# supabase/etl

Hardware: AMD Instinct MI355X
Metric: WAL bytes/s decoded (higher is better)
Workload: dtype u8; 1 GPU; cfg2_fixed_5xint4: 64 MiB batches of CopyData-framed pgoutput, device-resident in / device-resident out, offsets sidecar, NO_CONTROL | ASYNC; batch_bytes=67108819, frames_per_batch=594511, pool_batches=6, parallelism=shard1

## Files before the change

### etl_amd/csrc/plan.hip

```cpp
#include "lookback.hip.h"

namespace etlg {

struct WinLds {
  const ETLG_LDS_AS u8* base;
  DEV uint32_t w(uint32_t aoff) const { return ETLG_LDS_LD32(base + aoff); }
};
struct WinGlb {
  const u8* base; uint32_t lim;
  DEV uint32_t w(uint32_t aoff) const {
    uint32_t v = 0;
    if (aoff + 4 <= lim) __builtin_memcpy(&v, base + aoff, 4);
    else for (uint32_t k = 0; aoff + k < lim; k++) v |= (uint32_t)base[aoff + k] << (8 * k);
    return v;
  }
};
template <class M> DEV uint32_t rd32(const M& m, uint32_t off) {
  const uint32_t a = off & ~3u, s = off & 3u;
  return __builtin_amdgcn_alignbyte(m.w(a + 4), m.w(a), s);
}
template <class M> DEV uint64_t rd64(const M& m, uint32_t off) {
  const uint32_t a = off & ~3u, s = off & 3u;
  const uint32_t w0 = m.w(a), w1 = m.w(a + 4), w2 = m.w(a + 8);
  return __builtin_amdgcn_alignbyte(w1, w0, s) | ((uint64_t)__builtin_amdgcn_alignbyte(w2, w1, s) << 32);
// ... 10 lines not shown
  const int32_t sh = (int32_t)k - (int32_t)(4 * j);
  const uint32_t part = 0xFFFFFFFFu << (8 * ((uint32_t)sh & 3u));
  const uint32_t keep = sh <= 0 ? 0xFFFFFFFFu : sh >= 4 ? 0u : part;
  return (w & keep) | (0x30303030u & ~keep);
}

template <class M>
DEV uint64_t plan_int(const M& m, uint32_t cs, uint32_t n, uint32_t c0, uint32_t cls, uint32_t& ok) {
  const uint32_t neg = c0 == '-' ? 1u : 0u;
  const uint32_t sg = (c0 == '-' || c0 == '+') ? 1u : 0u;
  const uint32_t nd = n - sg;
  uint32_t bad = 0;
  uint64_t mag;
  if (cls == ETLG_TC_I64) {
    const uint32_t nn = n < 20u ? n : 20u;
    const uint32_t s0 = cs + nn - 20u, a = s0 & ~3u, s = s0 & 3u, k = 20u - (nd < 20u ? nd : 20u);
    const uint32_t w0 = m.w(a), w1 = m.w(a + 4), w2 = m.w(a + 8), w3 = m.w(a + 12), w4 = m.w(a + 16), w5 = m.w(a + 20);
    const uint32_t d0 = dig4(pad_word(__builtin_amdgcn_alignbyte(w1, w0, s), k, 0), bad);
    const uint32_t d1 = dig4(pad_word(__builtin_amdgcn_alignbyte(w2, w1, s), k, 1), bad);
    const uint32_t d2 = dig4(pad_word(__builtin_amdgcn_alignbyte(w3, w2, s), k, 2), bad);
    const uint32_t d3 = dig4(pad_word(__builtin_amdgcn_alignbyte(w4, w3, s), k, 3), bad);
    const uint32_t d4 = dig4(pad_word(__builtin_amdgcn_alignbyte(w5, w4, s), k, 4), bad);
    mag = (uint64_t)(d0 * 10000u + d1) * 1000000000000ull + (uint64_t)(d2 * 10000u + d3) * 10000ull + d4;
    const uint64_t lim = neg ? (1ull << 63) : (1ull << 63) - 1;
    ok = (n != 0u) & (nd != 0u) & (n <= 20u) & (nd <= 19u) & (bad == 0u) & (mag <= lim);
  } else {
    const uint32_t nn = n < 12u ? n : 12u;
    const uint32_t s0 = cs + nn - 12u, a = s0 & ~3u, s = s0 & 3u, k = 12u - (nd < 12u ? nd : 12u);
    const uint32_t w0 = m.w(a), w1 = m.w(a + 4), w2 = m.w(a + 8), w3 = m.w(a + 12);
    const uint32_t d0 = dig4(pad_word(__builtin_amdgcn_alignbyte(w1, w0, s), k, 0), bad);
    const uint32_t d1 = dig4(pad_word(__builtin_amdgcn_alignbyte(w2, w1, s), k, 1), bad);
    const uint32_t d2 = dig4(pad_word(__builtin_amdgcn_alignbyte(w3, w2, s), k, 2), bad);
    mag = (uint64_t)d0 * 100000000ull + (d1 * 10000u + d2);
    uint64_t lim;
    if (cls == ETLG_TC_U32) lim = 0xFFFFFFFFull;
    else if (cls == ETLG_TC_I16) lim = neg ? 0x8000ull : 0x7FFFull;
    else lim = neg ? 0x80000000ull : 0x7FFFFFFFull;
    ok = (n != 0u) & (nd != 0u) & (n <= 12u) & (nd <= 11u) & (bad == 0u) & (mag <= lim) & ((cls != ETLG_TC_U32) | (neg ^ 1u));
  }
  return neg ? 0 - mag : mag;
}

DEV int plan_find(const PlanParams& q, uint32_t rel_u) {
  const ETLG_CONST_AS uint32_t* t = (const ETLG_CONST_AS uint32_t*)(uintptr_t)q.tabs;
  int lo = 0, hi = (int)q.n_tabs - 1;
  while (lo <= hi) {
    const int mid = (lo + hi) >> 1;
    const uint32_t v = t[mid * (int)(sizeof(PlanTab) / 4)];
    if (v == rel_u) return mid;
    if (v < rel_u) lo = mid + 1; else hi = mid - 1;
  }
  return -1;
}

#define WSTAMP(k) do { if ((q.dbg & 64u) && threadIdx.x == 0) ((unsigned long long*)p.heap)[(size_t)blockIdx.x * 8 + (k)] = wall_clock64(); } while (0)
#define PSTAMP(k) do { if ((q.dbg & 32u) && threadIdx.x == 0 && (blockIdx.x & 15u) == 3u) { const unsigned long long t_ = clock64(); atomicAdd(&p.res->dbg_t[k], t_ - tprev); tprev = t_; } } while (0)

constexpr uint32_t kPreBeginLen = kBodyOff + 20u, kPreCommitLen = kBodyOff + 25u;
constexpr int kPreTilesPerWave = 8, kPreWaves = 8;
constexpr uint32_t pre_log2(uint32_t v) { return v <= 1u ? 0u : 1u + pre_log2(v >> 1); }
constexpr uint32_t kPreGroupLog = pre_log2(kPreTilesPerWave * kPreWaves);
static_assert((1u << kPreGroupLog) == (uint32_t)(kPreTilesPerWave * kPreWaves), "a group of the pre-pass is a power of two of tiles");
static_assert(kPreTilesPerWave <= 32 && kPreWaves <= 8, "cand_m / short_m are 32-bit masks; at most two waves per SIMD");
constexpr uint32_t kPlanMaxPolls = 1u << 15;

struct PlanPre2 { unsigned long long a0 = 0, l0 = 0, a1 = 0, l1 = 0; bool valid = false; };
struct PlanFold { uint32_t fx, mk, l0, l1; };
DEV PlanFold fold_id() { return PlanFold{0u, 0u, 0u, 0u}; }
DEV PlanFold fold_f(const PlanFold& a, const PlanFold& b) {
  return PlanFold{a.fx + b.fx, a.mk > b.mk ? a.mk : b.mk, b.mk ? b.l0 : a.l0, b.mk ? b.l1 : a.l1};
}
// ... 54 lines not shown
  const PlanFold own = fold_of(agg, tile_lsn);
  const PlanFold group_agg = fold_f(local, own);
  if (j == 63u && lane == 0) ETLG_ST_PAIR(g2 + 2 * (size_t)g, ST_AGG | fold_agg(group_agg), ST_AGG | fold_lsn(group_agg));
  PlanFold acc = fold_id();
  int64_t base = (int64_t)g - 1;
  for (;;) {
    const int64_t idx = base - 63 + (int64_t)lane;
    unsigned long long wa = ST_INCL, wl = ST_INCL;
    if (idx >= 0) {
      if (pre_valid) { wa = a1p; wl = l1p; }
      else ETLG_LD_PAIR(g2 + 2 * idx, wa, wl);
    }
    pre_valid = false;
    const unsigned long long st = pair_state(wa, wl);
    const unsigned long long m_incl = __ballot(st == ST_INCL);
    const unsigned long long m_empty = __ballot(st == 0);
    const int first_incl = m_incl ? 63 - __builtin_clzll(m_incl) : -1;
    const unsigned long long needed = first_incl <= 0 ? ~0ull : (~0ull << first_incl);
    if (m_empty & needed) {
      if (++polls > kPlanMaxPolls) { if (lane == 0) atomicOr(fail, 1u); return; }
      __builtin_amdgcn_s_sleep(2);
      continue;
    }
    const PlanFold wfold = fold_lane63(fold_scan((int)lane >= (first_incl < 0 ? 0 : first_incl) ? fold_of(wa, wl) : fold_id()));
    acc = fold_f(wfold, acc);
    if (first_incl >= 0) break;
    base -= 64;
  }
  if (j == 63u && lane == 0) { const PlanFold incl = fold_f(acc, group_agg); ETLG_ST_PAIR(g2 + 2 * (size_t)g, ST_INCL | fold_agg(incl), ST_INCL | fold_lsn(incl)); }
  const PlanFold r = fold_f(acc, local);
  ex = fold_agg(r); ex_lsn = fold_lsn(r);
}

template <int RD>
struct PlanLocal {
  uint32_t tbl, slot_id, pm, x_fx, fixed_dw, vbytes, bad;
  uint32_t tagf;
  uint64_t wal_start, b_lsn;
  uint32_t* rimg;
  uint32_t row[RD];
  uint64_t ord;
  uint64_t agg, tile_lsn, ex, ex_lsn, tile_pre_lsn;
  uint32_t tot_mark, tot_fx;
  bool early, done;
};

template <class M, int RD>
DEV void plan_local(const DecParams& p, const PlanParams& q, const M& m, u8* rows, bool stage_own, uint32_t a0, uint32_t tile, uint32_t nt, uint32_t my_o,
                    uint32_t span0, uint32_t span1, unsigned long long& tprev, PlanLocal<RD>& L, bool keep) {
  L.done = true;
  const uint32_t lane = threadIdx.x;
  const bool live = lane < nt;
  const uint32_t f = tile * 64u + lane;
  uint32_t* failp = &p.res->fused_fail;
  uint32_t bad = 0;

  const uint32_t o0 = my_o;
  const uint32_t o1 = (uint32_t)__builtin_amdgcn_update_dpp((int)span1, (int)my_o, 0x130, 0xF, 0xF, false);
  const uint32_t flen = o1 - o0;
  const uint32_t sane = (live ? 1u : 0u) & (o1 > o0) & (o0 >= span0) & (o1 <= span1) & (flen >= 38u);
  bad |= (live ? 1u : 0u) & (sane ^ 1u);
  const uint32_t fr = sane ? o0 - a0 : 0u;
  const uint64_t h30 = rd64(m, fr + 30);
  const uint32_t tag = (uint32_t)(h30 & 0xFF);
  const uint32_t rel = __builtin_bswap32((uint32_t)(h30 >> 8));
  const uint32_t ncols = ((uint32_t)(h30 >> 48) & 0xFFu) << 8 | (uint32_t)(h30 >> 56);
  bad |= sane & (uint32_t)(tag != 'I' && tag != 'U' && tag != 'D' && tag != 'B' && tag != 'C');
  const bool isD = sane && tag == 'D';
  const bool isI = sane && (tag == 'I' || tag == 'U'), isB = sane && tag == 'B', isC = sane && tag == 'C';
  int ti = -1;
  uint32_t row_dw = 0, slot_id = 0, want_cols = 0, key_dw = 0, n_ident = 0;
  {
    unsigned long long todo = __ballot(isI || isD);
    while (todo) {
      const int leader = __builtin_ctzll(todo);
      const uint32_t rel_u = (uint32_t)__builtin_amdgcn_readlane((int)rel, leader);
      const int t_u = plan_find(q, rel_u);
      const bool mine = (isI || isD) && rel == rel_u;
      if (t_u >= 0) {
        const ETLG_CONST_AS uint32_t* tw = (const ETLG_CONST_AS uint32_t*)(uintptr_t)(q.tabs + t_u);
        const uint32_t s_u = tw[1], n_u = tw[2], r_u = tw[3], k_u = tw[5], i_u = tw[6];
        if (mine) { ti = t_u; slot_id = s_u; want_cols = n_u; row_dw = r_u; key_dw = k_u; n_ident = i_u; }
      }
      todo &= ~__ballot(mine);
    }
  }
  bad |= (uint32_t)(isI && (ti < 0 || ncols != want_cols));
  bad |= (uint32_t)(isD && (ti < 0 || key_dw == 0 || (ncols != n_ident && ncols != want_cols)));
  uint64_t b_lsn = 0;
  if (isB) b_lsn = bswap64(rd64(m, fr + 31));
  if (isC) b_lsn = bswap64(rd64(m, fr + 32));
  const uint32_t fixed_dw = isI ? row_dw : isD ? key_dw : isB ? 2u : isC ? 4u : 0u;
  const uint32_t mark = isB ? (((f + 1) << 1) | 1u) : isC ? ((f + 1) << 1) : 0u;
  const uint32_t im = wave_scan_max(mark);
  const uint32_t pm = (uint32_t)__builtin_amdgcn_update_dpp(0, (int)im, 0x138, 0xF, 0xF, false);
  const uint32_t ifx = wave_scan_add(fixed_dw);
  const uint32_t tot_mark = wave_last(im), tot_fx = wave_last(ifx);
  const uint32_t x_fx = ifx - fixed_dw;
  uint64_t tile_lsn = 0;
  if (tot_mark & 1u) {
    const int src = (int)((tot_mark >> 1) - 1u - tile * 64u);
    tile_lsn = ((uint64_t)(uint32_t)__builtin_amdgcn_readlane((int)(uint32_t)(b_lsn >> 32), src) << 32) | (uint32_t)__builtin_amdgcn_readlane((int)(uint32_t)b_lsn, src);
    bad |= (uint32_t)((tile_lsn >> 62) != 0);
    tile_lsn &= ~(3ull << 62);
  }
  PSTAMP(2);
  WSTAMP(2);
  if (q.dbg & 4u) { if (tot_mark + tot_fx == 0xFFFFFFF1u) atomicOr(failp, 2u); return; }

  const uint64_t agg = ((uint64_t)tot_mark << 32) | tot_fx;
  const bool early = (tile & 63u) == 63u;
  uint64_t ex = 0, ex_lsn = 0;
  if (q.pre) bad |= (uint32_t)((isB && flen != kPreBeginLen) || (isC && flen != kPreCommitLen) || (isI && ti >= 0 && (row_dw != q.pre_row_dw || flen < q.pre_key_below)) ||
                               (isD && ti >= 0 && (key_dw != q.pre_key_dw || (flen >= q.pre_key_below && flen > q.pre_key_max))));
  else plan_publish2(q.desc, tile, agg, tile_lsn);
  if (early && !q.pre) plan_resolve2(q.desc, q.desc + 2 * (size_t)q.ntiles, tile, agg, tile_lsn, failp, PlanPre2(), ex, ex_lsn);
  {
    const uint64_t h0 = rd64(m, fr);
    const uint32_t len = __builtin_bswap32((uint32_t)(h0 >> 8));
    const uint32_t env = ((uint32_t)(h0 & 0xFF) == 'd') & (len + 1u == flen) & ((uint32_t)((h0 >> 40) & 0xFF) == 'w');
    const uint32_t shape = (tag == 'I' || tag == 'U') ? (uint32_t)((uint32_t)((h30 >> 40) & 0xFF) == 'N')
                         : tag == 'D' ? (uint32_t)((uint32_t)((h30 >> 40) & 0xFF) == 'K')
                         : tag == 'B' ? (uint32_t)(flen >= kBodyOff + 20) : (uint32_t)(flen >= kBodyOff + 25);
    bad |= sane & ((env & shape) ^ 1u);
  }
  const uint64_t wal_start = bswap64(rd64(m, fr + 6));
  uint64_t b_ts = 0, c_end = 0;
  uint32_t b_xid = 0, c_flags = 0;
  if (isB) { b_ts = bswap64(rd64(m, fr + 39)); b_xid = __builtin_bswap32(rd32(m, fr + 47)); }
  if (isC) { c_flags = (uint32_t)(h30 >> 8) & 0xFFu; c_end = bswap64(rd64(m, fr + 40)); b_ts = bswap64(rd64(m, fr + 48)); }
  uint32_t* rimg = q.lds_bytes > q.rows_off ? (uint32_t*)(rows + q.rows_off) + x_fx : (uint32_t*)(rows + (stage_own ? ((fr + 3u) & ~3u) : lane * 32u));
  if (isB && !bad) { rimg[0] = (uint32_t)b_ts; rimg[1] = (uint32_t)(b_ts >> 32); }
  if (isC && !bad) { rimg[0] = (uint32_t)c_end; rimg[1] = (uint32_t)(c_end >> 32); rimg[2] = (uint32_t)b_ts; rimg[3] = (uint32_t)(b_ts >> 32); }
  uint32_t vbytes = 0;
  if (!(q.dbg & 8u)) {
    unsigned long long todo = __ballot(isI && !bad);
    while (todo) {
      const int leader = __builtin_ctzll(todo);
      const int t_u = __builtin_amdgcn_readlane(ti, leader);
      const bool mine = isI && !bad && ti == t_u;
      const ETLG_CONST_AS uint32_t* tw = (const ETLG_CONST_AS uint32_t*)(uintptr_t)(q.tabs + t_u);
      const uint32_t n_u = tw[2], cb_u = tw[4];
      const ETLG_CONST_AS uint32_t* cw = (const ETLG_CONST_AS uint32_t*)(uintptr_t)(q.cols + cb_u);
      if (mine) {
        uint32_t cur = fr + 38;
        const uint32_t e = fr + flen;
        uint32_t acc = 0, cbad = 0;
        uint32_t cd_next = cw[0];
        for (uint32_t i = 0; i < n_u; i++) {
          const uint32_t cd = cd_next;
          cd_next = cw[i + 1 < n_u ? i + 1 : i];
          const uint32_t cls = cd & 0xFFu;
          uint32_t* slot = rimg + (cd >> 18);
          const uint32_t rc = cur < e ? cur : fr;
          const uint64_t ch = rd64(m, rc);
          const uint32_t kind = (uint32_t)(ch & 0xFF);
          const uint32_t len = __builtin_bswap32((uint32_t)(ch >> 8));
          const uint32_t c0 = (uint32_t)(ch >> 40) & 0xFFu;
          const uint32_t is_t = kind == 't', is_n = kind == 'n';
          const uint32_t fits = (cur < e) & (is_n | (is_t & (rc + 5 <= e) & (len <= e - rc - 5)));
          const uint32_t tl = (is_t & fits) ? len : 0u;
          uint32_t okv;
          uint64_t v;
          if (cls == ETLG_TC_BOOL) {
            okv = (tl == 1u) & ((c0 == 't') | (c0 == 'f'));
            v = c0 == 't';
          } else {
            v = plan_int(m, rc + 5, tl, c0, cls, okv);
          }
          const uint32_t good = fits & ((is_n & ((cd >> 8) & 1u)) | (is_t & okv));
          cbad |= good ^ 1u;
          const uint64_t val = is_t ? v : 0ull;
          slot[0] = (uint32_t)val;
          if (cls == ETLG_TC_I64) slot[1] = (uint32_t)(val >> 32);
          acc |= (is_n ? (uint32_t)ETLG_CELL_NULL : (uint32_t)ETLG_CELL_VALUE) << (2 * (i & 15));
          if ((i & 15) == 15 || i + 1 == n_u) { rimg[i >> 4] = acc; acc = 0; }
          vbytes += tl;
          cur = rc + (is_t ? 5u + tl : 1u);
        }
        bad |= cbad;
      }
      todo &= ~__ballot(mine);
    }
    unsigned long long todo_d = __ballot(isD && !bad);
    while (todo_d) {
      const int leader = __builtin_ctzll(todo_d);
      const int t_u = __builtin_amdgcn_readlane(ti, leader);
      const bool mine = isD && !bad && ti == t_u;
      const ETLG_CONST_AS uint32_t* tw = (const ETLG_CONST_AS uint32_t*)(uintptr_t)(q.tabs + t_u);
      const uint32_t n_u = tw[2], cb_u = tw[4], ni_u = tw[6], kb_u = tw[7];
      const ETLG_CONST_AS uint32_t* cw = (const ETLG_CONST_AS uint32_t*)(uintptr_t)(q.cols + cb_u);
      const ETLG_CONST_AS uint32_t* kw = (const ETLG_CONST_AS uint32_t*)(uintptr_t)(q.cols + kb_u);
      if (mine) {
        const bool dense = ncols != n_u;
        uint32_t cur = fr + 38;
        const uint32_t e = fr + flen;
        uint32_t acc = 0, cbad = 0;
        for (uint32_t i = 0; i < n_u; i++) {
          const uint32_t cd = cw[i], kd = kw[i];
          const uint32_t ident = kd & 1u;
          if (!ident && dense) continue;
          const uint32_t cls = cd & 0xFFu;
          const uint32_t rc = cur < e ? cur : fr;
          const uint64_t ch = rd64(m, rc);
          const uint32_t kind = (uint32_t)(ch & 0xFF);
          const uint32_t len = __builtin_bswap32((uint32_t)(ch >> 8));
          const uint32_t c0 = (uint32_t)(ch >> 40) & 0xFFu;
          const uint32_t is_t = kind == 't', is_n = kind == 'n';
          const uint32_t fits = (cur < e) & (is_n | (is_t & (rc + 5 <= e) & (len <= e - rc - 5)));
          const uint32_t tl = (is_t & fits) ? len : 0u;
          if (ident) {
            uint32_t okv;
            uint64_t v;
            if (cls == ETLG_TC_BOOL) { okv = (tl == 1u) & ((c0 == 't') | (c0 == 'f')); v = c0 == 't'; }
            else v = plan_int(m, rc + 5, tl, c0, cls, okv);
            const uint32_t good = fits & ((is_n & ((cd >> 8) & 1u)) | (is_t & okv));
            cbad |= good ^ 1u;
            const uint64_t val = is_t ? v : 0ull;
            uint32_t* slot = rimg + (kd >> 24);
            const uint32_t k = (kd >> 8) & 0xFFFFu;
            slot[0] = (uint32_t)val;
            if (cls == ETLG_TC_I64) slot[1] = (uint32_t)(val >> 32);
            acc |= (is_n ? (uint32_t)ETLG_CELL_NULL : (uint32_t)ETLG_CELL_VALUE) << (2 * (k & 15));
            if ((k & 15) == 15 || k + 1 == ni_u) { rimg[k >> 4] = acc; acc = 0; }
          } else {
            cbad |= fits ^ 1u;
          }
          vbytes += tl;
          cur = rc + (is_t ? 5u + tl : 1u);
        }
        bad |= cbad;
      }
      todo_d &= ~__ballot(mine);
    }
  }
  PSTAMP(3);
  WSTAMP(3);
  L.tbl = isB ? b_xid : (isI || isD) ? rel : 0u; L.slot_id = (isI || isD) ? slot_id : 0u; L.pm = pm; L.x_fx = x_fx; L.fixed_dw = fixed_dw; L.vbytes = vbytes; L.bad = bad;
  if (isD) c_flags = ETLG_OLD_KEY;
  L.tagf = tag | (c_flags << 8) | (((isI || isD) ? 1u : 0u) << 16) | ((isB ? 1u : 0u) << 17) | ((isC ? 1u : 0u) << 18) | ((live ? 1u : 0u) << 19);
  L.wal_start = wal_start; L.b_lsn = b_lsn; L.rimg = rimg;
  if (keep) {
#pragma unroll
    for (int d = 0; d < RD; d++) L.row[d] = rimg[d];
  }
  L.agg = agg; L.tile_lsn = tile_lsn; L.ex = ex; L.ex_lsn = ex_lsn; L.tot_mark = tot_mark; L.tot_fx = tot_fx; L.early = early; L.done = false;
}

DEV void plan_late_carry(DecParams& p, uint32_t* failp) {
  if (!(p.flags & 16u) || !p.carry) return;
  for (uint32_t polls = 0;; polls++) {
    if (__hip_atomic_load(&p.carry->carry_ready, __ATOMIC_ACQUIRE, __HIP_MEMORY_SCOPE_AGENT)) break;
    if (polls > kPlanMaxPolls) { if (threadIdx.x == 0) atomicOr(failp, 1u); break; }
    __builtin_amdgcn_s_sleep(8);
  }
  p.in_txn = __hip_atomic_load(&p.carry->out_in_txn, __ATOMIC_RELAXED, __HIP_MEMORY_SCOPE_AGENT);
  p.final_lsn = __hip_atomic_load(&p.carry->out_final_lsn, __ATOMIC_RELAXED, __HIP_MEMORY_SCOPE_AGENT);
  p.next_ord = __hip_atomic_load(&p.carry->out_next_ord, __ATOMIC_RELAXED, __HIP_MEMORY_SCOPE_AGENT);
  p.flags &= ~16u;
}

struct PlanPreWords { unsigned long long g0 = 0, g1 = 0, t0 = 0, t1 = 0; };
DEV PlanPreWords plan_pre_load(const PlanParams& q, uint32_t tile) {
  PlanPreWords w;
  if (q.pre && tile < q.ntiles) {
    const ETLG_CONST_AS unsigned long long* dt = (const ETLG_CONST_AS unsigned long long*)(uintptr_t)(q.pre + 2 * (size_t)tile);
    const ETLG_CONST_AS unsigned long long* dg = (const ETLG_CONST_AS unsigned long long*)(uintptr_t)(q.pre + 2 * ((size_t)q.ntiles + (tile >> kPreGroupLog)));
    w.t0 = dt[0]; w.t1 = dt[1]; w.g0 = dg[0]; w.g1 = dg[1];
  }
  return w;
}

template <int RD>
DEV void plan_resolve(DecParams& p, const PlanParams& q, uint32_t tile, PlanLocal<RD>& L, unsigned long long& tprev, const PlanPre2& pre = PlanPre2(), const PlanPreWords& pw = PlanPreWords()) {
  if (L.done) return;
  const uint32_t lane = threadIdx.x;
  const uint32_t f = tile * 64u + lane;
  uint32_t* failp = &p.res->fused_fail;
  uint32_t bad = L.bad;
  const bool isI = (L.tagf >> 16) & 1u, isB = (L.tagf >> 17) & 1u, isC = (L.tagf >> 18) & 1u;
  const uint32_t pm = L.pm;
  const uint64_t b_lsn = L.b_lsn;
  uint64_t ex = L.ex, ex_lsn = L.ex_lsn;

  if (q.pre) {
    const PlanFold r = fold_f(fold_of(pw.g0, pw.g1), fold_of(pw.t0, pw.t1));
    ex = fold_agg(r); ex_lsn = fold_lsn(r);
  }
  else if (!L.early) plan_resolve2(q.desc, q.desc + 2 * (size_t)q.ntiles, tile, L.agg, L.tile_lsn, failp, pre, ex, ex_lsn);
  PSTAMP(7);
  uint32_t pre_mark = (uint32_t)(ex >> 32);
  if (pre_mark == 0) {
    plan_late_carry(p, failp);
    if (p.in_txn) { pre_mark = 1u; ex |= 1ull << 32; }
  }
  const uint64_t pre_lsn = (pre_mark & 1u) && (pre_mark >> 1) != 0 ? ex_lsn : p.final_lsn;
  PSTAMP(4);
  WSTAMP(4);

  const uint32_t last = pre_mark > pm ? pre_mark : pm;
  const bool in_txn = (last & 1u) != 0;
  const uint32_t fb1 = last >> 1;
  uint64_t final_lsn = 0;
  {
    const bool here = in_txn && fb1 != 0 && fb1 - 1 >= tile * 64u;
    const uint32_t src = here ? fb1 - 1 - tile * 64u : 0u;
    const uint32_t lo = (uint32_t)__shfl((int)(uint32_t)b_lsn, (int)src, 64), hi = (uint32_t)__shfl((int)(uint32_t)(b_lsn >> 32), (int)src, 64);
    if (in_txn) final_lsn = here ? (((uint64_t)hi << 32) | lo) : pre_lsn;
  }
  uint64_t ord = 0;
  if (!isB && in_txn) ord = fb1 == 0 ? p.next_ord + f : (uint64_t)(f - (fb1 - 1));
  bad |= (uint32_t)((isI || isC) && !in_txn);
  bad |= (uint32_t)(isC && in_txn && b_lsn != final_lsn);
  L.bad = bad; L.ex = ex; L.tile_pre_lsn = pre_lsn;
  L.b_lsn = isI ? final_lsn : b_lsn;
  L.ord = ord;
}

template <bool REGS, int RD>
DEV void plan_store(DecParams& p, const PlanParams& q, uint32_t tile, const PlanLocal<RD>& L, unsigned long long& tprev) {
  if (L.done) return;
  const uint32_t lane = threadIdx.x;
  const uint32_t f = tile * 64u + lane;
  uint32_t* failp = &p.res->fused_fail;
  const uint32_t bad = L.bad;
  const uint32_t tag = L.tagf & 0xFFu, c_flags = (L.tagf >> 8) & 0xFFu;
  const bool live = (L.tagf >> 19) & 1u;
  const uint32_t x_fx = L.x_fx, fixed_dw = L.fixed_dw, vbytes = L.vbytes, tot_mark = L.tot_mark, tot_fx = L.tot_fx;
  const uint64_t tile_lsn = L.tile_lsn, pre_lsn = L.tile_pre_lsn;
  const uint32_t pre_mark = (uint32_t)(L.ex >> 32);
  const uint64_t pre_fx = (uint64_t)(uint32_t)L.ex << 2;

  if (tile == q.ntiles - 1 && lane == 0) {
    DevResult* r = p.res;
    r->n_events = p.nframes; r->fixed_bytes = pre_fx + ((uint64_t)tot_fx << 2); r->heap_bytes = 0; r->n_frames = p.nframes;
    const uint32_t lm = pre_mark > tot_mark ? pre_mark : tot_mark;
    const bool it = (lm & 1u) != 0;
    r->out_in_txn = it;
    uint64_t fl = 0, no = 0;
    if (it) {
      const uint32_t lb1 = lm >> 1;
      fl = tot_mark ? tile_lsn : pre_lsn;
      no = lb1 == 0 ? p.next_ord + p.nframes : (uint64_t)(p.nframes - (lb1 - 1));
    }
    r->out_final_lsn = fl; r->out_next_ord = no;
    __hip_atomic_store(&r->carry_ready, 1u, __ATOMIC_RELEASE, __HIP_MEMORY_SCOPE_AGENT);
  }

  const uint64_t fx_off = pre_fx + ((uint64_t)x_fx << 2);
  const uint32_t any_bad = __any(bad != 0u) ? 1u : 0u;
  const bool cap_ok = pre_fx + ((uint64_t)tot_fx << 2) <= p.fixed_cap;
  if (!any_bad && cap_ok && !(q.dbg & 8u)) {
    uint32_t* dst = (uint32_t*)(p.fixed + fx_off);
    if (REGS) {
#pragma unroll
      for (uint32_t d = 0; d < (uint32_t)RD; d++) if (d < fixed_dw) dst[d] = L.row[d];
    } else {
      const uint32_t* rimg = L.rimg;
      for (uint32_t d = 0; d < fixed_dw; d++) dst[d] = rimg[d];
    }
  }
  PSTAMP(5);
  if (live && !any_bad && cap_ok && !(q.dbg & 16u)) {
    p.ev_kind[f] = (u8)tag;
    p.ev_flags[f] = (u8)c_flags;
    p.ev_table[f] = L.tbl;
    p.ev_slot[f] = L.slot_id;
    p.ev_start[f] = L.wal_start;
    p.ev_commit[f] = L.b_lsn;
    p.ev_ord[f] = L.ord;
    p.ev_body[f] = fx_off;
  }
  PSTAMP(6);
  WSTAMP(5);
  const bool is_upd = (L.tagf & 0xFFu) == 'U', is_del = (L.tagf & 0xFFu) == 'D';
  const uint32_t pay = wave_last(wave_scan_add((is_upd || is_del) ? 0u : vbytes));
  if (lane == 0 && pay) atomicAdd(&p.res->pay_shard[tile & 31][0], (unsigned long long)pay);
  if (__ballot(is_upd && vbytes != 0)) {
    const uint32_t payu = wave_last(wave_scan_add(is_upd ? vbytes : 0u));
    if (lane == 0 && payu) atomicAdd(&p.res->pay_shard[tile & 31][1], (unsigned long long)payu);
  }
  if (__ballot(is_del && vbytes != 0)) {
    const uint32_t payd = wave_last(wave_scan_add(is_del ? vbytes : 0u));
    if (lane == 0 && payd) atomicAdd(&p.res->pay_shard[tile & 31][2], (unsigned long long)payd);
  }
  if ((any_bad || !cap_ok) && lane == 0) atomicOr(failp, 2u);
}

struct TileSpan { uint32_t nt, span0, span1, my_o; };
DEV TileSpan plan_span(const DecParams& p, uint32_t tile) {
  const uint32_t lane = threadIdx.x;
  TileSpan t;
  const uint32_t f0 = tile * 64u;
  t.nt = p.nframes - f0 < 64u ? p.nframes - f0 : 64u;
  const ETLG_CONST_AS uint32_t* offs_c = (const ETLG_CONST_AS uint32_t*)(uintptr_t)p.offs;
  t.span0 = offs_c[f0]; t.span1 = offs_c[f0 + t.nt];
  t.my_o = lane < t.nt ? p.offs[f0 + lane] : t.span1;
  return t;
}

template <int RD>
DEV void plan_stage_local(DecParams& p, const PlanParams& q, u8* smem, uint32_t tile, const TileSpan& ts, unsigned long long& tprev, PlanLocal<RD>& L, bool keep) {
  const uint32_t lane = threadIdx.x;
  L.done = true;
  const uint32_t nt = ts.nt, span0 = ts.span0, span1 = ts.span1, my_o = ts.my_o;
  PSTAMP(0);
  const uint32_t a0 = span0 & ~15u;
  const bool staged = span1 > span0 && span1 <= p.in_len && (uint64_t)(span1 - a0) + 64 <= q.rows_off && !(q.dbg & 1u);
  if (staged) {
    const uint32_t npieces = (span1 - a0 + 1023u) >> 10;
    for (uint32_t k = 0; k < npieces; k++) {
      const uint32_t c = a0 + (k << 10) + (lane << 4);
      if (c < span1 && (uint64_t)c + 16 <= p.in_len) ETLG_GLDS16(p.in + c, smem + (k << 10));
    }
    const uint32_t tail = a0 + (((uint32_t)p.in_len - a0) & ~15u);
    if (tail < span1 && (uint64_t)tail + 16 > p.in_len && tail + lane < p.in_len && lane < 16) smem[tail - a0 + lane] = p.in[tail + lane];
    ETLG_VMEM_WAIT();
    PSTAMP(1);
    WSTAMP(1);
    if (q.dbg & 2u) { if (smem[lane * 97u] == 0xEE && smem[lane * 13u + 5u] == 0xEF && my_o == 0xFFFFFFF1u) atomicOr(&p.res->fused_fail, 2u); return; }
    const WinLds m{(const ETLG_LDS_AS u8*)smem};
    plan_local(p, q, m, smem, true, a0, tile, nt, my_o, span0, span1, tprev, L, keep);
  } else {
    const WinGlb m{p.in, (uint32_t)p.in_len};
    plan_local(p, q, m, smem, false, 0u, tile, nt, my_o, span0, span1, tprev, L, keep);
  }
}

DEV bool plan_frames_from_device(DecParams& p, PlanParams& q) {
  if (!p.nframes_dev) return true;
  const ETLG_CONST_AS uint32_t* r = (const ETLG_CONST_AS uint32_t*)(uintptr_t)p.nframes_dev;
  const uint32_t nf = r[0], flags = r[1] | r[2];
  if (flags != 0 || nf == 0 || nf > p.nframes) {
    if (blockIdx.x == 0 && threadIdx.x == 0) {
      atomicOr(&p.res->fused_fail, 32u);
      __hip_atomic_store(&p.res->carry_ready, 1u, __ATOMIC_RELEASE, __HIP_MEMORY_SCOPE_AGENT);
    }
    return false;
  }
  p.nframes = nf;
  q.ntiles = (nf + 63u) >> 6;
  return true;
}

template <bool TWO, int RD>
DEV void plan_kernel(DecParams& p, const PlanParams& q_in, u8* smem) {
  PlanParams q = q_in;
  const uint32_t lane = threadIdx.x;
  unsigned long long tprev = (q.dbg & 32u) ? clock64() : 0ull;
  const uint32_t tile = blockIdx.x;
  WSTAMP(0);
  if (q.clear_words) {
    const uint32_t per = (q.clear_words + gridDim.x - 1) / gridDim.x;
    for (uint32_t i = lane; i < per; i += 64) { const uint32_t w = blockIdx.x * per + i; if (w < q.clear_words) q.d_clear[w] = 0; }
  }
  if (!(p.flags & 16u) && !load_carry(p)) return;
  if (!plan_frames_from_device(p, q)) return;
  const uint32_t t0 = TWO ? 2u * blockIdx.x : blockIdx.x;
  if (t0 >= q.ntiles) return;
  const TileSpan sa = plan_span(p, t0);
  const PlanPreWords pwa = plan_pre_load(q, t0), pwb = TWO ? plan_pre_load(q, t0 + 1u) : PlanPreWords();
  TileSpan sb = sa;
  if (TWO && t0 + 1u < q.ntiles) sb = plan_span(p, t0 + 1u);
  PlanLocal<RD> A;
  plan_stage_local(p, q, smem, t0, sa, tprev, A, TWO);
  if (TWO) {
    const uint32_t t1 = t0 + 1u;
    PlanLocal<RD> B;
    B.done = true;
    if (t1 < q.ntiles) {
      __threadfence_block();
      __syncthreads();
      plan_stage_local(p, q, smem, t1, sb, tprev, B, false);
    }
    PlanPre2 preA, preB;
    if (!A.done && !A.early && !q.pre) preA = plan_prefetch2(q.desc, q.desc + 2 * (size_t)q.ntiles, t0);
    if (!B.done && !B.early && !q.pre) preB = plan_prefetch2(q.desc, q.desc + 2 * (size_t)q.ntiles, t1);
    plan_resolve(p, q, t0, A, tprev, preA, pwa);
    plan_resolve(p, q, t1, B, tprev, preB, pwb);
    plan_store<true>(p, q, t0, A, tprev);
    plan_store<false>(p, q, t1, B, tprev);
  } else {
    plan_resolve(p, q, t0, A, tprev, PlanPre2(), pwa);
    plan_store<false>(p, q, t0, A, tprev);
  }
}

__global__ __launch_bounds__(kPreWaves * 64) void k_plan_pre(DecParams p, PlanParams q) {
  __shared__ unsigned long long s_wagg[kPreWaves][2];
  if (!plan_frames_from_device(p, q)) return;
  if (blockIdx.x >= ((q.ntiles + (1u << kPreGroupLog) - 1u) >> kPreGroupLog)) return;
  const uint32_t lane = threadIdx.x & 63u, wave = (uint32_t)__builtin_amdgcn_readfirstlane((int)(threadIdx.x >> 6)), g = blockIdx.x;
  const uint32_t t0 = (g << kPreGroupLog) + wave * (uint32_t)kPreTilesPerWave;
  uint32_t o[kPreTilesPerWave + 1];
#pragma unroll
  for (int i = 0; i <= kPreTilesPerWave; i++) {
    const uint64_t f = (uint64_t)(t0 + (uint32_t)i) * 64u + lane;
    o[i] = p.offs[f < p.nframes ? f : p.nframes];
  }
  uint32_t cand_m = 0;
  uint32_t short_m = 0;
  uint32_t tagv[kPreTilesPerWave];
  uint64_t lsnv[kPreTilesPerWave];
#pragma unroll
  for (int i = 0; i < kPreTilesPerWave; i++) {
    const uint64_t f = (uint64_t)(t0 + (uint32_t)i) * 64u + lane;
    const uint32_t o0 = o[i];
    const uint32_t nxt = (uint32_t)__builtin_amdgcn_readfirstlane((int)o[i + 1]);
    const uint32_t o1 = (uint32_t)__builtin_amdgcn_update_dpp((int)nxt, (int)o0, 0x130, 0xF, 0xF, false);
    const uint32_t flen = o1 - o0;
    const bool cand = f < p.nframes && o1 > o0 && o1 <= p.in_len && (flen == kPreBeginLen || flen == kPreCommitLen || (flen >= q.pre_key_below && flen <= q.pre_key_max));
    tagv[i] = 0; lsnv[i] = 0;
    if (cand) { cand_m |= 1u << i; tagv[i] = p.in[o0 + 30] | (flen << 8); lsnv[i] = ld_be64(p.in + o0 + 31); }
    if (flen < q.pre_key_below) short_m |= 1u << i;
  }
  PlanFold run = fold_id();
  PlanFold keep = fold_id();
// ... 44 lines not shown
  if (lane == 0) {
    const PlanFold all = fold_f(before, run);
    ETLG_ST_PAIR(gd + 2 * (size_t)g, tagbits | fold_agg(all), tagbits | fold_lsn(all));
    ticket = atomicAdd(q.pre_ticket, 1u);
  }
  ticket = (uint32_t)__builtin_amdgcn_readfirstlane((int)ticket);
  if (ticket != ng - 1u) return;
  PlanFold carry = fold_id();
  unsigned long long na = 0, nl = 0;
  if (lane < ng) ETLG_LD_PAIR(gd + 2 * (size_t)lane, na, nl);
  for (uint32_t base = 0; base < ng; base += 64u) {
    const uint32_t gi = base + lane;
    unsigned long long a = gi < ng ? na : tagbits, l = gi < ng ? nl : tagbits;
    if (gi + 64u < ng) ETLG_LD_PAIR(gd + 2 * (size_t)(gi + 64u), na, nl);
    bool have = pair_state(a, l) == tagbits;
    bool gave_up = false;
    for (uint32_t polls = 0;; polls++) {
      if (!have) { ETLG_LD_PAIR(gd + 2 * (size_t)gi, a, l); have = pair_state(a, l) == tagbits; }
      if (!__ballot(!have)) break;
      if (polls > kPlanMaxPolls) { if (lane == 0) atomicOr(&p.res->fused_fail, 1u); gave_up = true; break; }
      __builtin_amdgcn_s_sleep(2);
    }
    const PlanFold inc = fold_scan(gi < ng ? fold_of(a, l) : fold_id());
    PlanFold exc;
    exc.fx = (uint32_t)__builtin_amdgcn_update_dpp(0, (int)inc.fx, 0x138, 0xF, 0xF, false); exc.mk = (uint32_t)__builtin_amdgcn_update_dpp(0, (int)inc.mk, 0x138, 0xF, 0xF, false);
    exc.l0 = (uint32_t)__builtin_amdgcn_update_dpp(0, (int)inc.l0, 0x138, 0xF, 0xF, false); exc.l1 = (uint32_t)__builtin_amdgcn_update_dpp(0, (int)inc.l1, 0x138, 0xF, 0xF, false);
    const PlanFold r = fold_f(carry, exc);
    if (gi < ng && !gave_up) { gd[2 * (size_t)gi] = fold_agg(r); gd[2 * (size_t)gi + 1] = fold_lsn(r); }
    carry = fold_f(carry, fold_lane63(inc));
  }
  if (lane == 0) __hip_atomic_store(q.pre_ticket, 0u, __ATOMIC_RELAXED, __HIP_MEMORY_SCOPE_AGENT);
}

__global__ __launch_bounds__(64, ETLG_PLAN_MINWAVES) void k_plan(DecParams p, PlanParams q) {
  ETLG_DYNAMIC_LDS(smem);
  plan_kernel<false, 1>(p, q, smem);
}

template <int RD>
__global__ __launch_bounds__(64, ETLG_PLAN_MINWAVES) void k_plan2(DecParams p, PlanParams q) {
  ETLG_DYNAMIC_LDS(smem);
  plan_kernel<true, RD>(p, q, smem);
}

}

extern "C" {

using namespace etlg;

void etlg_k_launch_plan_pre(const DecParams* p, const void* qv, hipStream_t s) {
  const PlanParams* q = (const PlanParams*)qv;
  hipLaunchKernelGGL(k_plan_pre, dim3((q->ntiles + (1u << kPreGroupLog) - 1u) >> kPreGroupLog), dim3(kPreWaves * 64), 0, s, *p, *q);
}

void etlg_k_launch_plan(const DecParams* p, const void* qv, hipStream_t s) {
  const PlanParams* q = (const PlanParams*)qv;
  if (q->lds_bytes == q->rows_off && q->max_row_dw <= 8u && !(q->dbg & 512u)) {
    if (q->max_row_dw <= 6u) hipLaunchKernelGGL(k_plan2<6>, dim3((q->ntiles + 1) / 2), dim3(64), q->lds_bytes, s, *p, *q);
    else hipLaunchKernelGGL(k_plan2<8>, dim3((q->ntiles + 1) / 2), dim3(64), q->lds_bytes, s, *p, *q);
  } else hipLaunchKernelGGL(k_plan, dim3(q->ntiles), dim3(64), q->lds_bytes, s, *p, *q);
}

uint32_t etlg_k_plan_pre_group_log(void) { return kPreGroupLog; }

int etlg_k_plan_set_lds(void) {
  const int a = hipFuncSetAttribute((const void*)k_plan, hipFuncAttributeMaxDynamicSharedMemorySize, 64 * 1024) == hipSuccess ? 0 : 1;
  const int b = hipFuncSetAttribute((const void*)k_plan2<6>, hipFuncAttributeMaxDynamicSharedMemorySize, 64 * 1024) == hipSuccess ? 0 : 1;
  const int c = hipFuncSetAttribute((const void*)k_plan2<8>, hipFuncAttributeMaxDynamicSharedMemorySize, 64 * 1024) == hipSuccess ? 0 : 1;
  return a | b | c;
}

}
```

Measured before the change: 1860 GB/s.

## Add pure-insert tile fast path, direct fixed-row writes, and hook-free kernel variants

Adds a fast path for 64-frame tiles made entirely of inserts into one relation: it skips the begin/commit LSN reads, the mark and fixed-size wave scans, and the delete loop, and computes row offsets directly from the row width. When a prefix-sum sidecar exists, the single-tile kernel writes rows straight into the global fixed buffer instead of staging them in LDS and copying them out later. Debug hooks are compiled out through template specialisations, so the default launch carries no timing or stamp branches. The int-range check is also made branchless. The cost is more template instantiations and code size, plus a capacity check that is now done before any row is written.

Result: slower. 1841 GB/s (-1.0%).

```diff
diff --git a/etl_amd/csrc/plan.hip b/etl_amd/csrc/plan.hip
--- a/etl_amd/csrc/plan.hip
+++ b/etl_amd/csrc/plan.hip
@@ -66,11 +66,10 @@
     const uint32_t d1 = dig4(pad_word(__builtin_amdgcn_alignbyte(w2, w1, s), k, 1), bad);
     const uint32_t d2 = dig4(pad_word(__builtin_amdgcn_alignbyte(w3, w2, s), k, 2), bad);
     mag = (uint64_t)d0 * 100000000ull + (d1 * 10000u + d2);
-    uint64_t lim;
-    if (cls == ETLG_TC_U32) lim = 0xFFFFFFFFull;
-    else if (cls == ETLG_TC_I16) lim = neg ? 0x8000ull : 0x7FFFull;
-    else lim = neg ? 0x80000000ull : 0x7FFFFFFFull;
-    ok = (n != 0u) & (nd != 0u) & (n <= 12u) & (nd <= 11u) & (bad == 0u) & (mag <= lim) & ((cls != ETLG_TC_U32) | (neg ^ 1u));
+    const uint32_t has_sign = cls != ETLG_TC_U32 ? 1u : 0u;
+    const uint32_t lim_pos = cls == ETLG_TC_U32 ? 0xFFFFFFFFu : cls == ETLG_TC_I16 ? 0x7FFFu : 0x7FFFFFFFu;
+    const uint32_t lim = lim_pos + (neg & has_sign);
+    ok = (n != 0u) & (nd != 0u) & (n <= 12u) & (nd <= 11u) & (bad == 0u) & (mag <= (uint64_t)lim) & (has_sign | (neg ^ 1u));
   }
   return neg ? 0 - mag : mag;
 }
@@ -191,6 +190,17 @@
   ex = fold_agg(r); ex_lsn = fold_lsn(r);
 }
 
+struct PlanPreWords { unsigned long long g0 = 0, g1 = 0, t0 = 0, t1 = 0; };
+DEV PlanPreWords plan_pre_load(const PlanParams& q, uint32_t tile) {
+  PlanPreWords w;
+  if (q.pre && tile < q.ntiles) {
+    const ETLG_CONST_AS unsigned long long* dt = (const ETLG_CONST_AS unsigned long long*)(uintptr_t)(q.pre + 2 * (size_t)tile);
+    const ETLG_CONST_AS unsigned long long* dg = (const ETLG_CONST_AS unsigned long long*)(uintptr_t)(q.pre + 2 * ((size_t)q.ntiles + (tile >> kPreGroupLog)));
+    w.t0 = dt[0]; w.t1 = dt[1]; w.g0 = dg[0]; w.g1 = dg[1];
+  }
+  return w;
+}
+
 template <int RD>
 struct PlanLocal {
   uint32_t tbl, slot_id, pm, x_fx, fixed_dw, vbytes, bad;
@@ -202,11 +212,12 @@
   uint64_t agg, tile_lsn, ex, ex_lsn, tile_pre_lsn;
   uint32_t tot_mark, tot_fx;
   bool early, done;
+  bool pure;
 };
 
-template <class M, int RD>
+template <class M, int RD, bool TWO, bool DIRECT>
 DEV void plan_local(const DecParams& p, const PlanParams& q, const M& m, u8* rows, bool stage_own, uint32_t a0, uint32_t tile, uint32_t nt, uint32_t my_o,
-                    uint32_t span0, uint32_t span1, unsigned long long& tprev, PlanLocal<RD>& L, bool keep) {
+                    uint32_t span0, uint32_t span1, unsigned long long& tprev, PlanLocal<RD>& L, bool keep, const PlanPreWords& pw) {
   L.done = true;
   const uint32_t lane = threadIdx.x;
   const bool live = lane < nt;
@@ -246,22 +257,29 @@
   }
   bad |= (uint32_t)(isI && (ti < 0 || ncols != want_cols));
   bad |= (uint32_t)(isD && (ti < 0 || key_dw == 0 || (ncols != n_ident && ncols != want_cols)));
+  const bool pure = !TWO && nt == 64u && __ballot(isI && rel == (uint32_t)__builtin_amdgcn_readfirstlane((int)rel)) == ~0ull;
   uint64_t b_lsn = 0;
-  if (isB) b_lsn = bswap64(rd64(m, fr + 31));
-  if (isC) b_lsn = bswap64(rd64(m, fr + 32));
   const uint32_t fixed_dw = isI ? row_dw : isD ? key_dw : isB ? 2u : isC ? 4u : 0u;
-  const uint32_t mark = isB ? (((f + 1) << 1) | 1u) : isC ? ((f + 1) << 1) : 0u;
-  const uint32_t im = wave_scan_max(mark);
-  const uint32_t pm = (uint32_t)__builtin_amdgcn_update_dpp(0, (int)im, 0x138, 0xF, 0xF, false);
-  const uint32_t ifx = wave_scan_add(fixed_dw);
-  const uint32_t tot_mark = wave_last(im), tot_fx = wave_last(ifx);
-  const uint32_t x_fx = ifx - fixed_dw;
+  uint32_t pm = 0, tot_mark = 0, tot_fx, x_fx;
   uint64_t tile_lsn = 0;
-  if (tot_mark & 1u) {
-    const int src = (int)((tot_mark >> 1) - 1u - tile * 64u);
-    tile_lsn = ((uint64_t)(uint32_t)__builtin_amdgcn_readlane((int)(uint32_t)(b_lsn >> 32), src) << 32) | (uint32_t)__builtin_amdgcn_readlane((int)(uint32_t)b_lsn, src);
-    bad |= (uint32_t)((tile_lsn >> 62) != 0);
-    tile_lsn &= ~(3ull << 62);
+  if (pure) {
+    const uint32_t r_u = (uint32_t)__builtin_amdgcn_readfirstlane((int)row_dw);
+    x_fx = lane * r_u; tot_fx = 64u * r_u;
+  } else {
+    if (isB) b_lsn = bswap64(rd64(m, fr + 31));
+    if (isC) b_lsn = bswap64(rd64(m, fr + 32));
+    const uint32_t mark = isB ? (((f + 1) << 1) | 1u) : isC ? ((f + 1) << 1) : 0u;
+    const uint32_t im = wave_scan_max(mark);
+    pm = (uint32_t)__builtin_amdgcn_update_dpp(0, (int)im, 0x138, 0xF, 0xF, false);
+    const uint32_t ifx = wave_scan_add(fixed_dw);
+    tot_mark = wave_last(im); tot_fx = wave_last(ifx);
+    x_fx = ifx - fixed_dw;
+    if (tot_mark & 1u) {
+      const int src = (int)((tot_mark >> 1) - 1u - tile * 64u);
+      tile_lsn = ((uint64_t)(uint32_t)__builtin_amdgcn_readlane((int)(uint32_t)(b_lsn >> 32), src) << 32) | (uint32_t)__builtin_amdgcn_readlane((int)(uint32_t)b_lsn, src);
+      bad |= (uint32_t)((tile_lsn >> 62) != 0);
+      tile_lsn &= ~(3ull << 62);
+    }
   }
   PSTAMP(2);
   WSTAMP(2);
@@ -286,13 +304,25 @@
   const uint64_t wal_start = bswap64(rd64(m, fr + 6));
   uint64_t b_ts = 0, c_end = 0;
   uint32_t b_xid = 0, c_flags = 0;
-  if (isB) { b_ts = bswap64(rd64(m, fr + 39)); b_xid = __builtin_bswap32(rd32(m, fr + 47)); }
-  if (isC) { c_flags = (uint32_t)(h30 >> 8) & 0xFFu; c_end = bswap64(rd64(m, fr + 40)); b_ts = bswap64(rd64(m, fr + 48)); }
-  uint32_t* rimg = q.lds_bytes > q.rows_off ? (uint32_t*)(rows + q.rows_off) + x_fx : (uint32_t*)(rows + (stage_own ? ((fr + 3u) & ~3u) : lane * 32u));
-  if (isB && !bad) { rimg[0] = (uint32_t)b_ts; rimg[1] = (uint32_t)(b_ts >> 32); }
-  if (isC && !bad) { rimg[0] = (uint32_t)c_end; rimg[1] = (uint32_t)(c_end >> 32); rimg[2] = (uint32_t)b_ts; rimg[3] = (uint32_t)(b_ts >> 32); }
+  if (!pure) {
+    if (isB) { b_ts = bswap64(rd64(m, fr + 39)); b_xid = __builtin_bswap32(rd32(m, fr + 47)); }
+    if (isC) { c_flags = (uint32_t)(h30 >> 8) & 0xFFu; c_end = bswap64(rd64(m, fr + 40)); b_ts = bswap64(rd64(m, fr + 48)); }
+  }
+  uint32_t* rimg;
+  bool room = true;
+  if (DIRECT) {
+    const uint64_t pre_fx = (uint64_t)fold_f(fold_of(pw.g0, pw.g1), fold_of(pw.t0, pw.t1)).fx << 2;
+    room = pre_fx + ((uint64_t)tot_fx << 2) <= p.fixed_cap;
+    rimg = (uint32_t*)(p.fixed + pre_fx) + x_fx;
+  } else {
+    rimg = q.lds_bytes > q.rows_off ? (uint32_t*)(rows + q.rows_off) + x_fx : (uint32_t*)(rows + (stage_own ? ((fr + 3u) & ~3u) : lane * 32u));
+  }
+  if (!pure && room) {
+    if (isB && !bad) { rimg[0] = (uint32_t)b_ts; rimg[1] = (uint32_t)(b_ts >> 32); }
+    if (isC && !bad) { rimg[0] = (uint32_t)c_end; rimg[1] = (uint32_t)(c_end >> 32); rimg[2] = (uint32_t)b_ts; rimg[3] = (uint32_t)(b_ts >> 32); }
+  }
   uint32_t vbytes = 0;
-  if (!(q.dbg & 8u)) {
+  if (!(q.dbg & 8u) && room) {
     unsigned long long todo = __ballot(isI && !bad);
     while (todo) {
       const int leader = __builtin_ctzll(todo);
@@ -341,7 +371,7 @@
       }
       todo &= ~__ballot(mine);
     }
-    unsigned long long todo_d = __ballot(isD && !bad);
+    unsigned long long todo_d = pure ? 0ull : __ballot(isD && !bad);
     while (todo_d) {
       const int leader = __builtin_ctzll(todo_d);
       const int t_u = __builtin_amdgcn_readlane(ti, leader);
@@ -398,8 +428,8 @@
   L.tbl = isB ? b_xid : (isI || isD) ? rel : 0u; L.slot_id = (isI || isD) ? slot_id : 0u; L.pm = pm; L.x_fx = x_fx; L.fixed_dw = fixed_dw; L.vbytes = vbytes; L.bad = bad;
   if (isD) c_flags = ETLG_OLD_KEY;
   L.tagf = tag | (c_flags << 8) | (((isI || isD) ? 1u : 0u) << 16) | ((isB ? 1u : 0u) << 17) | ((isC ? 1u : 0u) << 18) | ((live ? 1u : 0u) << 19);
-  L.wal_start = wal_start; L.b_lsn = b_lsn; L.rimg = rimg;
-  if (keep) {
+  L.wal_start = wal_start; L.b_lsn = b_lsn; L.rimg = rimg; L.pure = pure;
+  if (!DIRECT && keep) {
 #pragma unroll
     for (int d = 0; d < RD; d++) L.row[d] = rimg[d];
   }
@@ -419,18 +449,7 @@
   p.flags &= ~16u;
 }
 
-struct PlanPreWords { unsigned long long g0 = 0, g1 = 0, t0 = 0, t1 = 0; };
-DEV PlanPreWords plan_pre_load(const PlanParams& q, uint32_t tile) {
-  PlanPreWords w;
-  if (q.pre && tile < q.ntiles) {
-    const ETLG_CONST_AS unsigned long long* dt = (const ETLG_CONST_AS unsigned long long*)(uintptr_t)(q.pre + 2 * (size_t)tile);
-    const ETLG_CONST_AS unsigned long long* dg = (const ETLG_CONST_AS unsigned long long*)(uintptr_t)(q.pre + 2 * ((size_t)q.ntiles + (tile >> kPreGroupLog)));
-    w.t0 = dt[0]; w.t1 = dt[1]; w.g0 = dg[0]; w.g1 = dg[1];
-  }
-  return w;
-}
-
-template <int RD>
+template <int RD, bool TWO>
 DEV void plan_resolve(DecParams& p, const PlanParams& q, uint32_t tile, PlanLocal<RD>& L, unsigned long long& tprev, const PlanPre2& pre = PlanPre2(), const PlanPreWords& pw = PlanPreWords()) {
   if (L.done) return;
   const uint32_t lane = threadIdx.x;
@@ -457,26 +476,31 @@
   PSTAMP(4);
   WSTAMP(4);
 
-  const uint32_t last = pre_mark > pm ? pre_mark : pm;
-  const bool in_txn = (last & 1u) != 0;
-  const uint32_t fb1 = last >> 1;
-  uint64_t final_lsn = 0;
-  {
-    const bool here = in_txn && fb1 != 0 && fb1 - 1 >= tile * 64u;
-    const uint32_t src = here ? fb1 - 1 - tile * 64u : 0u;
-    const uint32_t lo = (uint32_t)__shfl((int)(uint32_t)b_lsn, (int)src, 64), hi = (uint32_t)__shfl((int)(uint32_t)(b_lsn >> 32), (int)src, 64);
-    if (in_txn) final_lsn = here ? (((uint64_t)hi << 32) | lo) : pre_lsn;
-  }
-  uint64_t ord = 0;
-  if (!isB && in_txn) ord = fb1 == 0 ? p.next_ord + f : (uint64_t)(f - (fb1 - 1));
-  bad |= (uint32_t)((isI || isC) && !in_txn);
-  bad |= (uint32_t)(isC && in_txn && b_lsn != final_lsn);
+  uint64_t final_lsn = 0, ord = 0;
+  if (!TWO && L.pure) {
+    const uint32_t fb1 = pre_mark >> 1;
+    if (pre_mark & 1u) { final_lsn = pre_lsn; ord = fb1 == 0 ? p.next_ord + f : (uint64_t)(f - (fb1 - 1)); }
+    else bad |= 1u;
+  } else {
+    const uint32_t last = pre_mark > pm ? pre_mark : pm;
+    const bool in_txn = (last & 1u) != 0;
+    const uint32_t fb1 = last >> 1;
+    {
+      const bool here = in_txn && fb1 != 0 && fb1 - 1 >= tile * 64u;
+      const uint32_t src = here ? fb1 - 1 - tile * 64u : 0u;
+      const uint32_t lo = (uint32_t)__shfl((int)(uint32_t)b_lsn, (int)src, 64), hi = (uint32_t)__shfl((int)(uint32_t)(b_lsn >> 32), (int)src, 64);
+      if (in_txn) final_lsn = here ? (((uint64_t)hi << 32) | lo) : pre_lsn;
+    }
+    if (!isB && in_txn) ord = fb1 == 0 ? p.next_ord + f : (uint64_t)(f - (fb1 - 1));
+    bad |= (uint32_t)((isI || isC) && !in_txn);
+    bad |= (uint32_t)(isC && in_txn && b_lsn != final_lsn);
+  }
   L.bad = bad; L.ex = ex; L.tile_pre_lsn = pre_lsn;
   L.b_lsn = isI ? final_lsn : b_lsn;
   L.ord = ord;
 }
 
-template <bool REGS, int RD>
+template <bool REGS, int RD, bool DIRECT>
 DEV void plan_store(DecParams& p, const PlanParams& q, uint32_t tile, const PlanLocal<RD>& L, unsigned long long& tprev) {
   if (L.done) return;
   const uint32_t lane = threadIdx.x;
@@ -509,7 +533,7 @@
   const uint64_t fx_off = pre_fx + ((uint64_t)x_fx << 2);
   const uint32_t any_bad = __any(bad != 0u) ? 1u : 0u;
   const bool cap_ok = pre_fx + ((uint64_t)tot_fx << 2) <= p.fixed_cap;
-  if (!any_bad && cap_ok && !(q.dbg & 8u)) {
+  if (!DIRECT && !any_bad && cap_ok && !(q.dbg & 8u)) {
     uint32_t* dst = (uint32_t*)(p.fixed + fx_off);
     if (REGS) {
 #pragma unroll
@@ -558,8 +582,8 @@
   return t;
 }
 
-template <int RD>
-DEV void plan_stage_local(DecParams& p, const PlanParams& q, u8* smem, uint32_t tile, const TileSpan& ts, unsigned long long& tprev, PlanLocal<RD>& L, bool keep) {
+template <int RD, bool TWO, bool DIRECT>
+DEV void plan_stage_local(DecParams& p, const PlanParams& q, u8* smem, uint32_t tile, const TileSpan& ts, unsigned long long& tprev, PlanLocal<RD>& L, bool keep, const PlanPreWords& pw) {
   const uint32_t lane = threadIdx.x;
   L.done = true;
   const uint32_t nt = ts.nt, span0 = ts.span0, span1 = ts.span1, my_o = ts.my_o;
@@ -579,10 +603,10 @@
     WSTAMP(1);
     if (q.dbg & 2u) { if (smem[lane * 97u] == 0xEE && smem[lane * 13u + 5u] == 0xEF && my_o == 0xFFFFFFF1u) atomicOr(&p.res->fused_fail, 2u); return; }
     const WinLds m{(const ETLG_LDS_AS u8*)smem};
-    plan_local(p, q, m, smem, true, a0, tile, nt, my_o, span0, span1, tprev, L, keep);
+    plan_local<WinLds, RD, TWO, DIRECT>(p, q, m, smem, true, a0, tile, nt, my_o, span0, span1, tprev, L, keep, pw);
   } else {
     const WinGlb m{p.in, (uint32_t)p.in_len};
-    plan_local(p, q, m, smem, false, 0u, tile, nt, my_o, span0, span1, tprev, L, keep);
+    plan_local<WinGlb, RD, TWO, DIRECT>(p, q, m, smem, false, 0u, tile, nt, my_o, span0, span1, tprev, L, keep, pw);
   }
 }
 
@@ -602,9 +626,12 @@
   return true;
 }
 
-template <bool TWO, int RD>
+constexpr uint32_t kPlanDbgHooks = 127u;
+template <bool TWO, int RD, bool HOOKS, bool DIRECT>
 DEV void plan_kernel(DecParams& p, const PlanParams& q_in, u8* smem) {
+  static_assert(!(TWO && DIRECT), "two tiles share a window: the first one's rows wait in registers");
   PlanParams q = q_in;
+  if (!HOOKS) q.dbg &= ~kPlanDbgHooks;
   const uint32_t lane = threadIdx.x;
   unsigned long long tprev = (q.dbg & 32u) ? clock64() : 0ull;
   const uint32_t tile = blockIdx.x;
@@ -622,7 +649,7 @@
   TileSpan sb = sa;
   if (TWO && t0 + 1u < q.ntiles) sb = plan_span(p, t0 + 1u);
   PlanLocal<RD> A;
-  plan_stage_local(p, q, smem, t0, sa, tprev, A, TWO);
+  plan_stage_local<RD, TWO, DIRECT>(p, q, smem, t0, sa, tprev, A, TWO, pwa);
   if (TWO) {
     const uint32_t t1 = t0 + 1u;
     PlanLocal<RD> B;
@@ -630,18 +657,18 @@
     if (t1 < q.ntiles) {
       __threadfence_block();
       __syncthreads();
-      plan_stage_local(p, q, smem, t1, sb, tprev, B, false);
+      plan_stage_local<RD, TWO, DIRECT>(p, q, smem, t1, sb, tprev, B, false, pwb);
     }
     PlanPre2 preA, preB;
     if (!A.done && !A.early && !q.pre) preA = plan_prefetch2(q.desc, q.desc + 2 * (size_t)q.ntiles, t0);
     if (!B.done && !B.early && !q.pre) preB = plan_prefetch2(q.desc, q.desc + 2 * (size_t)q.ntiles, t1);
-    plan_resolve(p, q, t0, A, tprev, preA, pwa);
-    plan_resolve(p, q, t1, B, tprev, preB, pwb);
-    plan_store<true>(p, q, t0, A, tprev);
-    plan_store<false>(p, q, t1, B, tprev);
+    plan_resolve<RD, TWO>(p, q, t0, A, tprev, preA, pwa);
+    plan_resolve<RD, TWO>(p, q, t1, B, tprev, preB, pwb);
+    plan_store<true, RD, false>(p, q, t0, A, tprev);
+    plan_store<false, RD, false>(p, q, t1, B, tprev);
   } else {
-    plan_resolve(p, q, t0, A, tprev, PlanPre2(), pwa);
-    plan_store<false>(p, q, t0, A, tprev);
+    plan_resolve<RD, TWO>(p, q, t0, A, tprev, PlanPre2(), pwa);
+    plan_store<false, RD, DIRECT>(p, q, t0, A, tprev);
   }
 }
 
@@ -752,15 +779,16 @@
   if (lane == 0) __hip_atomic_store(q.pre_ticket, 0u, __ATOMIC_RELAXED, __HIP_MEMORY_SCOPE_AGENT);
 }
 
+template <bool HOOKS, bool DIRECT>
 __global__ __launch_bounds__(64, ETLG_PLAN_MINWAVES) void k_plan(DecParams p, PlanParams q) {
   ETLG_DYNAMIC_LDS(smem);
-  plan_kernel<false, 1>(p, q, smem);
-}
-
-template <int RD>
-__global__ __launch_bounds__(64, ETLG_PLAN_MINWAVES) void k_plan2(DecParams p, PlanParams q) {
+  plan_kernel<false, 1, HOOKS, DIRECT>(p, q, smem);
+}
+
+template <int RD, bool HOOKS>
+__global__ __launch_bounds__(64, HOOKS ? ETLG_PLAN_MINWAVES - 1 : ETLG_PLAN_MINWAVES) void k_plan2(DecParams p, PlanParams q) {
   ETLG_DYNAMIC_LDS(smem);
-  plan_kernel<true, RD>(p, q, smem);
+  plan_kernel<true, RD, HOOKS, false>(p, q, smem);
 }
 
 }
@@ -776,19 +804,25 @@
 
 void etlg_k_launch_plan(const DecParams* p, const void* qv, hipStream_t s) {
   const PlanParams* q = (const PlanParams*)qv;
+  const bool hooks = (q->dbg & kPlanDbgHooks) != 0;
+  const dim3 one(q->ntiles), two((q->ntiles + 1) / 2);
+#define ETLG_PLAN_LAUNCH(kernel, grid) hipLaunchKernelGGL(kernel, grid, dim3(64), q->lds_bytes, s, *p, *q)
   if (q->lds_bytes == q->rows_off && q->max_row_dw <= 8u && !(q->dbg & 512u)) {
-    if (q->max_row_dw <= 6u) hipLaunchKernelGGL(k_plan2<6>, dim3((q->ntiles + 1) / 2), dim3(64), q->lds_bytes, s, *p, *q);
-    else hipLaunchKernelGGL(k_plan2<8>, dim3((q->ntiles + 1) / 2), dim3(64), q->lds_bytes, s, *p, *q);
-  } else hipLaunchKernelGGL(k_plan, dim3(q->ntiles), dim3(64), q->lds_bytes, s, *p, *q);
+    if (q->max_row_dw <= 6u) { if (hooks) ETLG_PLAN_LAUNCH((k_plan2<6, true>), two); else ETLG_PLAN_LAUNCH((k_plan2<6, false>), two); }
+    else { if (hooks) ETLG_PLAN_LAUNCH((k_plan2<8, true>), two); else ETLG_PLAN_LAUNCH((k_plan2<8, false>), two); }
+  } else if (q->pre) { if (hooks) ETLG_PLAN_LAUNCH((k_plan<true, true>), one); else ETLG_PLAN_LAUNCH((k_plan<false, true>), one); }
+  else { if (hooks) ETLG_PLAN_LAUNCH((k_plan<true, false>), one); else ETLG_PLAN_LAUNCH((k_plan<false, false>), one); }
+#undef ETLG_PLAN_LAUNCH
 }
 
 uint32_t etlg_k_plan_pre_group_log(void) { return kPreGroupLog; }
 
 int etlg_k_plan_set_lds(void) {
-  const int a = hipFuncSetAttribute((const void*)k_plan, hipFuncAttributeMaxDynamicSharedMemorySize, 64 * 1024) == hipSuccess ? 0 : 1;
-  const int b = hipFuncSetAttribute((const void*)k_plan2<6>, hipFuncAttributeMaxDynamicSharedMemorySize, 64 * 1024) == hipSuccess ? 0 : 1;
-  const int c = hipFuncSetAttribute((const void*)k_plan2<8>, hipFuncAttributeMaxDynamicSharedMemorySize, 64 * 1024) == hipSuccess ? 0 : 1;
-  return a | b | c;
-}
-
-}
+  const void* ks[] = {(const void*)k_plan<false, false>, (const void*)k_plan<false, true>, (const void*)k_plan<true, false>, (const void*)k_plan<true, true>,
+                      (const void*)k_plan2<6, false>, (const void*)k_plan2<6, true>, (const void*)k_plan2<8, false>, (const void*)k_plan2<8, true>};
+  int bad = 0;
+  for (const void* k : ks) bad |= hipFuncSetAttribute(k, hipFuncAttributeMaxDynamicSharedMemorySize, 64 * 1024) == hipSuccess ? 0 : 1;
+  return bad;
+}
+
+}
```
